# zraorg/ZRA

Hardware: AMD Instinct MI355X
Metric: compress + RA-decompress GiB/s, 16 GiB @ 64 KiB frames, 1/2/4/8 MI355X (higher is better)
Workload: dtype u8

## Files before the change

### zra_amd/csrc/zra_decode.hip

```cpp
#include "zra_dev.h"
#include "zra_kernels.h"

using namespace zra_dev;

namespace {

constexpr int DEC_THREADS = 64;
constexpr int BATCH = 64;
#ifndef ZRA_XWIN
#define ZRA_XWIN 4032
#endif
constexpr u32 XPRE = 64, XWIN = ZRA_XWIN;
constexpr u32 BLOCK_MAX = 128u << 10;

__constant__ u32 c_ll_base[36] = {0,1,2,3,4,5,6,7,8,9,10,11,12,13,14,15,16,18,20,22,24,28,32,40,48,64,128,256,512,1024,2048,4096,8192,16384,32768,65536};
__constant__ u8 c_ll_bits[36] = {0,0,0,0,0,0,0,0,0,0,0,0,0,0,0,0,1,1,1,1,2,2,3,3,4,6,7,8,9,10,11,12,13,14,15,16};
__constant__ u32 c_ml_base[53] = {3,4,5,6,7,8,9,10,11,12,13,14,15,16,17,18,19,20,21,22,23,24,25,26,27,28,29,30,31,32,33,34,
                                  35,37,39,41,43,47,51,59,67,83,99,131,259,515,1027,2051,4099,8195,16387,32771,65539};
__constant__ u8 c_ml_bits[53] = {0,0,0,0,0,0,0,0,0,0,0,0,0,0,0,0,0,0,0,0,0,0,0,0,0,0,0,0,0,0,0,0,
                                 1,1,1,1,2,2,3,3,4,4,5,7,8,9,10,11,12,13,14,15,16};
__constant__ short c_ll_defnorm[36] = {4,3,2,2,2,2,2,2,2,2,2,2,2,1,1,1,2,2,2,2,2,2,2,2,2,3,2,1,1,1,1,1,-1,-1,-1,-1};
__constant__ short c_ml_defnorm[53] = {1,4,3,2,2,2,2,2,2,1,1,1,1,1,1,1,1,1,1,1,1,1,1,1,1,1,1,1,1,1,1,1,
                                       1,1,1,1,1,1,1,1,1,1,1,1,1,1,-1,-1,-1,-1,-1,-1,-1};
__constant__ short c_of_defnorm[29] = {1,1,1,1,1,1,2,2,2,1,1,1,1,1,1,1,1,1,1,1,1,1,1,1,-1,-1,-1,-1,-1};
__constant__ u16 c_huf_t0[16][2] = {{0,0},{0,0},{38,130},{448,128},{556,128},{714,128},{883,128},{897,128},{926,128},{947,128},{1107,128},{1177,128},{1242,128},{1349,128},{1455,128},{722,128}};
__constant__ u16 c_huf_t1[16][2] = {{1,1},{1,1},{1313,74},{1353,74},{1353,74},{1418,74},{1437,74},{1515,75},{1613,75},{1729,77},{2083,81},{2379,87},{2415,93},{2644,106},{2422,124},{1891,145}};

__device__ __forceinline__ u64 mk_seqsym(u32 baseValue, u32 addBits, u32 nbBits, u32 nextBase) {
  return (u64)baseValue | ((u64)addBits << 32) | ((u64)nbBits << 40) | ((u64)nextBase << 48);
}
__device__ __forceinline__ u32 mk_cell(u32 sym, u32 addBits, u32 nbBits, u32 nextBase) {
  return sym | (addBits << 8) | (nbBits << 16) | (nextBase << 20);
}

#ifdef ZRA_SMALL_PROFILE
__device__ unsigned long long zra_small_prof[64];
extern "C" __attribute__((visibility("default"))) void ZraHipDebugReadSmallProfile(unsigned long long* out16, int reset) {
  (void)hipMemcpyFromSymbol(out16, HIP_SYMBOL(zra_small_prof), sizeof(unsigned long long) * 64);
  if (reset) { unsigned long long z[64] = {0}; (void)hipMemcpyToSymbol(HIP_SYMBOL(zra_small_prof), z, sizeof(z)); }
}
#define SPROF(k) { __builtin_amdgcn_s_waitcnt(0); const u64 n_ = __builtin_amdgcn_s_memtime(); if (lane == 0) atomicAdd(&zra_small_prof[k], n_ - spt_); spt_ = n_; }
#define SPROF_T0 u64 spt_ = __builtin_amdgcn_s_memtime();
#define SPROF_RESET spt_ = __builtin_amdgcn_s_memtime();
#else
#define SPROF(k)
#define SPROF_T0
#define SPROF_RESET
#endif
#ifdef ZRA_SMALL_PROFILE
#define PPROF_T0 u64 ppt_ = __builtin_amdgcn_s_memtime();
#define PPROF(k) if (FUSED) { __builtin_amdgcn_s_waitcnt(0); const u64 n_ = __builtin_amdgcn_s_memtime(); if (lane == 0) atomicAdd(&zra_small_prof[k], n_ - ppt_); ppt_ = n_; }
#define LPROF_T0 u64 lpt_ = __builtin_amdgcn_s_memtime();
#define LPROF(k) { __builtin_amdgcn_s_waitcnt(0); const u64 n_ = __builtin_amdgcn_s_memtime(); atomicAdd(&zra_small_prof[k], n_ - lpt_); lpt_ = n_; }
#else
#define PPROF_T0
#define PPROF(k)
#define LPROF_T0
#define LPROF(k)
#endif
constexpr u32 STAGE_BYTES = 512;
struct __attribute__((aligned(16))) ParseShared {
  u8 w0[STAGE_BYTES + 16];
  u8 w1[STAGE_BYTES + 16];
  union {
    u64 wt[64];
    u32 stage[1024];
// ... 474 lines not shown
      u32 pos = endPos;
      if (fcsHave && (fcsHi != 0 || fcsLo != produced)) err = ZE_CORRUPTION;
      if (!err && hasChecksum) { if (srcSize - pos < 4) err = ZE_CHECKSUM_WRONG; else pos += 4; }
      if (!err && pos != srcSize) err = ZE_SRCSIZE_WRONG;
    }
    if (!err) {
      const u32 p0 = a.pieceBase[j], p1 = a.pieceBase[j + 1];
      for (u32 p = p0; p < p1; p++) {
        const ZraRaPiece q = a.pieces[p];
        const u32 have = q.srcOff >= produced ? 0u : min(q.len, produced - q.srcOff);
        if (have) copy_bytes(a.raOut + q.dstOff, a.out + a.outOff[j] + q.srcOff, have, lane, nthreads);
        if (have < q.len) fill_bytes(a.raOut + q.dstOff + have, 0, q.len - have, lane, nthreads);
      }
    }
  }
}

}

namespace {
template <bool FUSED, bool ALL = false>
__device__ __forceinline__ u32 parse_job(const ZraDecodeArgs& a, const u32 j, ParseShared& S, const int lane, u32* ldsT) {
  u32 outcome = 0;
  {
    const u64 so = a.frameOff[(size_t)j * a.offStride], se = a.frameOff[(size_t)j * a.offStride + 1];
    const u8* const src = a.body + so;
    const bool spanOk = se >= so && se <= a.bodySize;
    const u32 srcSize = spanOk ? (u32)(se - so) : 0u;
    u8* const dst = a.out + a.outOff[j];
    const u32 dstCap = a.outCap[j];
    const u32 limit = a.limit ? a.limit[j] : 0xFFFFFFFFu;
    ZraDecFrame* const F = &a.frames[j];
    u32 nBlk = 0; bool bail = false;
    const u32* prevT[3] = {nullptr, nullptr, nullptr};

    auto stage = [&](u8* w, u32 pos) -> u32 {
      const u32 avail = pos < srcSize ? min(srcSize - pos, STAGE_BYTES) : 0u;
      const u32 at = 8u * (u32)lane;
      u64 v = 0;
      if (at + 8 <= avail) v = ld64(src + pos + at);
      else for (u32 k = 0; at + k < avail && k < 8; k++) v |= (u64)src[pos + at + k] << (8 * k);
      *(u64*)(w + at) = v;
      if (lane < 2) *(u64*)(w + STAGE_BYTES + 8 * lane) = 0;
      return avail;
    };
    PPROF_T0
    const u32 startPos = a.round == 0 ? 0u : F->blkPos;
    const u32 staged0 = stage(S.w0, startPos);

    if (lane == 0) {
      S.err = 0; S.frameEnd = 0; S.winPos = startPos; S.winLen = staged0;
      if (a.round == 0) {
        S.produced = 0; S.hufValid = 0; S.llValid = S.mlValid = S.ofValid = 0; S.ofShare = 0;
        S.rep[0] = 1; S.rep[1] = 4; S.rep[2] = 8;
      }
    }
    wsync();
    if (lane == 0) {
      if (a.round == 0) {
        const u8* const hsrc = S.w0;
        u32 hs = 0;
        S.fcsHave = 0; S.hasChecksum = 0; S.bigWindow = 0;
        if (!spanOk || srcSize < 9) S.err = ZE_SRCSIZE_WRONG;
        else {
          u32 fhd = hsrc[4], did = fhd & 3, ss = (fhd >> 5) & 1, fcs = fhd >> 6;
          u32 didSize = did == 3 ? 4 : did;
          u32 fcsSize = fcs == 0 ? ss : fcs == 1 ? 2 : fcs == 2 ? 4 : 8;
// ... 120 lines not shown
      {
        const u32 at = bpos + S.seqPos;
        const u32 got = stage(S.w1, at);
        (void)got;
        wsync();
      }
      const u8* const sw = S.w1 - S.seqPos;
      const u8* const swLim = S.w1 + STAGE_BYTES + 8;
      if (lane == 0) {
        parse_seq_header(S, sw + S.seqPos, bsize - S.seqPos);
        if (S.err) { S.lateErr = S.err; S.err = 0; S.nbSeq = 0; S.seqTables = 0; }
        if (S.alloc && S.nbSeq) {
          const u64 take = ((u64)S.nbSeq + 3) & ~3ull;
          const u64 at = atomicAdd((unsigned long long*)&a.counters[ZRA_DC_SEQCUR], (unsigned long long)take);
          if (at + take > a.seqCap) S.alloc = 0;
          S.seqBase = at;
        }
      }
      wsync();
      if (ALL && (!S.alloc || nBlk >= a.bpf)) { bail = true; break; }
      if (!S.alloc) {
        if (lane == 0) {
          save_persistent(S.hdrPos, produced0, hv0, hmb0, hns0, hx20);
          if (!FUSED) a.nextActive[atomicAdd(&a.counters[ZRA_DC_NNEXT], 1u)] = j;
        }
        handed = true; outcome = 2;
        wsync();
        break;
      }

      PPROF(10)
      const u32 nbSeq = S.nbSeq, regen = S.litRegen;
      const size_t jb = ALL ? (size_t)j * a.bpf + nBlk : (size_t)j;
      u32* const T = ALL ? a.blkTables + jb * ZRA_DEC_TBL_WORDS : a.tables + (size_t)j * ZRA_DEC_TBL_WORDS;
      if (S.seqTables) {
        for (int kind = 0; kind < 3; kind++) {
          const int k = kind == 0 ? 0 : kind == 1 ? 2 : 1;
          const u32 mode = k == 0 ? (S.seqModes >> 6) : k == 2 ? ((S.seqModes >> 4) & 3) : ((S.seqModes >> 2) & 3);
          if (lane == 0) {
            u32 tl = 0, ms = 0, used = 0;
            seq_table_parse(S, k, mode, sw + S.seqPos, bsize - S.seqPos, &tl, &ms, &used, swLim);
            S.seqPos += used; S.tl = tl; S.ms = ms;
            if (mode == 3) { u32 v = k == 0 ? S.llValid : k == 1 ? S.mlValid : S.ofValid; if (!v) S.err = ZE_CORRUPTION; }
            if (S.err) { S.lateErr = S.err; S.err = 0; }
          }
          wsync();
          PPROF(11)
          if (S.lateErr) break;
          const u32 tl = S.tl, ms = S.ms;
          u32* const G = T + (k == 0 ? ZRA_DEC_TBL_LL : k == 1 ? ZRA_DEC_TBL_ML : ZRA_DEC_TBL_OF);
          if (mode == 1) {
            if (lane == 0) {
              if (k == 2) { G[0] = mk_cell(ms, ms, 0, 0); S.ofShare = (ms > 22) ? 256u : 0u; }
              else G[0] = mk_cell(ms, k == 0 ? c_ll_bits[ms] : c_ml_bits[ms], 0, 0);
              if (FUSED) { u32* const GL = ldsT + (k == 0 ? ZRA_LDS_TBL_LL : k == 1 ? ZRA_LDS_TBL_ML : ZRA_LDS_TBL_OF); GL[0] = G[0]; if (k != 2) GL[1] = k == 0 ? c_ll_base[ms] : c_ml_base[ms]; }
            }
          } else if (mode != 3) {
            build_fse_dtable(S.stage, S.norm, ms, tl, k, S.spread, (u64*)S.w0, S.wnext, lane);
            wsync();
            const u32 words = (k == 2 ? 1u : 2u) << tl;
            if (!FUSED) for (u32 i = lane; i < (1u << tl); i += DEC_THREADS) G[i] = S.stage[k == 2 ? i : 2 * i];
            if (FUSED) { u32* const GL = ldsT + (k == 0 ? ZRA_LDS_TBL_LL : k == 1 ? ZRA_LDS_TBL_ML : ZRA_LDS_TBL_OF); for (u32 i = lane; i < words; i += DEC_THREADS) GL[i] = S.stage[i]; }
            if (k == 2) {
              u32 cnt = 0;
              for (u32 i = lane; i < (1u << tl); i += DEC_THREADS) cnt += (S.stage[i] & 0xFF) > 22;
              cnt = wave_sum(cnt);
              if (lane == 0) S.ofShare = cnt << (8 - tl);
            }
            wsync();
          }
          if (lane == 0 && mode != 3) {
            if (k == 0) { S.llLog = tl; S.llValid = 1; } else if (k == 1) { S.mlLog = tl; S.mlValid = 1; } else { S.ofLog = tl; S.ofValid = 1; }
          }
          if (ALL) {
            if (mode == 3 && prevT[k] && prevT[k] != G) {
              const u32 lg = k == 0 ? S.llLog : k == 1 ? S.mlLog : S.ofLog;
              for (u32 i = lane; i < (1u << lg); i += DEC_THREADS) G[i] = prevT[k][i];
            }
            prevT[k] = G;
          }
          wsync();
          PPROF(12)
        }
      }

      if (ALL) {
        ZraDecFrame* const D = &a.blkRecs[jb];
        if (lane == 0) {
          save_persistent_to(D, S.hdrPos, produced0, S.hufValid, S.hufMaxBits, S.hufNSym, S.hufX2);
          if (nBlk) { D->rep[0] = ZRA_REP_MARK(0); D->rep[1] = ZRA_REP_MARK(1); D->rep[2] = ZRA_REP_MARK(2); }
          D->bpos = bpos; D->bsize = bsize; D->blast = S.blkLast;
          D->litKind = S.litKind; D->litRegen = regen; D->litArg = S.litArg; D->litBase = S.litBase;
          D->litStreams = S.litStreams;
          for (int k = 0; k < 4; k++) { D->streamOff[k] = S.streamOff[k]; D->streamLen[k] = S.streamLen[k]; }
          D->hufErr = 0; D->lateErr = S.lateErr;
          D->nbSeq = S.lateErr ? 0u : nbSeq; D->seqPos = S.seqPos; D->seqBase = S.seqBase;
          D->longMode = 0;
          D->chainErr = 0; D->nSeqValid = 0; D->seqOut = 0; D->seqLit = 0; D->truncated = 0;
          a.pending[atomicAdd(&a.counters[ZRA_DC_NPENDING], 1u)] = (u32)jb;
          if (S.litKind == 2) a.hufJobs[atomicAdd(&a.counters[ZRA_DC_NHUF], 1u)] = (u32)jb;
          S.produced = produced0 + (S.blkLast ? 0u : ZRA_FMB_BLOCK); S.blkPos = bpos + bsize; S.frameEnd = S.blkLast;
          S.winLen = 0;
        }
        if (S.litKind == 2) {
          for (u32 i = lane; i < 256; i += DEC_THREADS) { D->weights[i] = S.weights[i]; D->hufStart[i] = S.hufStart[i]; }
        }
        if (S.lateErr) bail = true;
        nBlk++;
        wsync();
        continue;
// ... 381 lines not shown
    bc += nb; return v;
  }
  __device__ __forceinline__ u32 read_fast(u32 nb) {
    const u32 v = (u32)((c << (bc & 63)) >> ((64 - nb) & 63));
    bc += nb; return v;
  }
  __device__ __forceinline__ int reload() {
    if (bc > 64) return OVERFLOW;
    if (ptr >= 8) { ptr -= bc >> 3; bc &= 7; c = fetch(ptr); return UNFINISHED; }
    if (ptr == 0) return bc < 64 ? ENDOFBUFFER : COMPLETED;
    u32 nbBytes = bc >> 3; int r = UNFINISHED;
    if (ptr < nbBytes) { nbBytes = ptr; r = ENDOFBUFFER; }
    ptr -= nbBytes; bc -= nbBytes * 8; c = fetch(ptr);
    return r;
  }
  __device__ __forceinline__ void reload_quiet(bool wide, const u8* pad) {
    const u32 nb = bc <= 64 ? min(bc >> 3, ptr) : 0u;
    ptr -= nb; bc -= nb * 8;
    const u64 v = RING ? fetch(ptr) : ld64(wide ? base + ptr : pad);
    c = nb ? v : c;
  }
};
typedef ZdsT<false> Zds;

}

namespace {
template <bool LDSTAB>
__device__ __forceinline__ void chain_body(const ZraDecodeArgs& a, u32* const ldsTabs, u32* const baseLL, u32* const baseML, u32* const ldsRings = nullptr) {
  const int lane = threadIdx.x;
  const u32 nPend = a.counters[ZRA_DC_NPENDING];
  bool have = false, drained = false;
  ZraDecFrame* F = nullptr;
  const u32* T = nullptr;
  u64* sq = nullptr;
  ZdsT<LDSTAB> br; br.c = 0; br.bc = 0; br.ptr = 0; br.base = nullptr; br.ring = nullptr; br.rLo = 0;
  br.lim = a.body + a.bodySize; br.pf = make_uint4(0, 0, 0, 0); br.pfState = 0; br.pfAge = 0;
  if (LDSTAB) br.ring = (u8*)(ldsRings + (u32)lane * CHAIN_RING_WORDS);
  u32 sLL = 0, sOF = 0, sML = 0, rep0 = 1, rep1 = 4, rep2 = 8;
  u32 i = 0, nbSeq = 0, outPos = 0, litPos = 0, outCap = 0, regen = 0, produced0 = 0, limit = 0;
  u32 longMode = 0, err = 0, jErr = 0xFFFFFFFFu, valid = 0, validOut = 0, validLit = 0, truncated = 0;
  u64 q0 = 0, q1 = 0, q2 = 0;
  u32 eL = 0, eM = 0, eO = 0;
  bool wide = false; const u8* pad = nullptr;
  bool fresh = false; u32 freshJob = 0;
  const u16* const cells16 = (const u16*)ldsTabs + (size_t)lane * ZRA_DEC_TBL_WORDS;
  u32 logLL = 0, logML = 0, logOF = 0;
  auto fetch_cells = [&]() {
    if (LDSTAB) { eL = cells16[ZRA_DEC_TBL_LL + sLL]; eM = cells16[ZRA_DEC_TBL_ML + sML]; eO = cells16[ZRA_DEC_TBL_OF + sOF]; }
    else { eL = T[ZRA_DEC_TBL_LL + sLL]; eM = T[ZRA_DEC_TBL_ML + sML]; eO = T[ZRA_DEC_TBL_OF + sOF]; }
  };
  auto c_code = [&](u32 e) -> u32 { return e & 63u; };
  auto c_sbits = [&](u32 e, u32 lg) -> u32 { if (LDSTAB) return lg - (31u - (u32)__builtin_clz(e >> 6)); return (e >> 16) & 0xF; };
  auto c_sbase = [&](u32 e, u32 lg) -> u32 {
    if (LDSTAB) { const u32 v = e >> 6, hb = 31u - (u32)__builtin_clz(v); return (v ^ (1u << hb)) << (lg - hb); }
    return e >> 20;
  };
  baseLL[lane] = lane < 36 ? c_ll_base[lane] | (LDSTAB ? (u32)c_ll_bits[lane] << 24 : 0u) : 0u;
  baseML[lane] = lane < 53 ? c_ml_base[lane] | (LDSTAB ? (u32)c_ml_bits[lane] << 24 : 0u) : 0u;
  wsync();
  if (LDSTAB && (u32)lane >= ZRA_CHAIN_LDS_FRAMES) drained = true;

  auto finish = [&]() {
    { const u32 r = valid & 3u, b = valid - r;
      if (r >= 1) sq[b] = q0;
      if (r >= 2) sq[b + 1] = q1;
      if (r >= 3) sq[b + 2] = q2; }
    if (!err && !truncated) {
      if (regen - litPos > outCap - outPos) err = ZE_DSTSIZE_TOOSMALL;
    }
    F->chainErr = err; F->nSeqValid = valid; F->seqOut = validOut; F->seqLit = validLit; F->truncated = truncated;
    F->repOut[0] = rep0; F->repOut[1] = rep1; F->repOut[2] = rep2;
    have = false;
  };

  for (;;) {
    const u64 want = __ballot(!have && !drained);
    if (want) {
      u32 base = 0;
      const u32 cnt = (u32)__builtin_popcountll(want);
      if (lane == (int)__builtin_ctzll(want)) base = atomicAdd(&a.counters[ZRA_DC_QCHAIN], cnt);
      base = bcast_u32(base, (u32)__builtin_ctzll(want));
      if (!have && !drained) {
        const u32 idx = base + (u32)__builtin_popcountll(want & ((1ull << lane) - 1ull));
        if (idx >= nPend) drained = true;
        else {
          const u32 j = a.pending[idx];
          const size_t gj = frame_of(a, j);
          F = &a.frames[j];
          T = a.tables + (size_t)j * ZRA_DEC_TBL_WORDS;
          const u8* const blk = a.body + a.frameOff[gj * a.offStride] + F->bpos;
          nbSeq = F->nbSeq; regen = F->litRegen; produced0 = F->produced; longMode = F->longMode;
          outCap = a.outCap[gj] - produced0;
          limit = a.limit ? a.limit[gj] : 0xFFFFFFFFu;
          sq = a.seqs + F->seqBase;
          rep0 = F->rep[0]; rep1 = F->rep[1]; rep2 = F->rep[2];
          i = 0; outPos = 0; litPos = 0; err = 0; jErr = 0xFFFFFFFFu; valid = 0; validOut = 0; validLit = 0; truncated = 0;
          have = true; br.rLo = 0; br.pfState = 0;
          if (F->hufErr) { err = ZE_CORRUPTION; nbSeq = 0; finish(); }
          else if (F->lateErr) { err = F->lateErr; nbSeq = 0; finish(); }
          else if (nbSeq) {
            if (!br.init(blk + F->seqPos, F->bsize - F->seqPos)) { err = ZE_CORRUPTION; finish(); }
            else {
              logLL = F->llLog; logOF = F->ofLog; logML = F->mlLog;
              sLL = br.read(logLL); br.reload();
              sOF = br.read(logOF); br.reload();
              sML = br.read(logML); br.reload();
              wide = F->bsize - F->seqPos >= 8;
              pad = a.body + a.frameOff[gj * a.offStride];
              if (LDSTAB) { fresh = true; freshJob = j; } else fetch_cells();
            }
          }
        }
      }
    }
    if (LDSTAB) {
      u64 nm = __ballot(fresh);
      while (nm) {
        const u32 l = (u32)__builtin_ctzll(nm); nm &= nm - 1;
        const u32 jj = bcast_u32(freshJob, l);
        const uint4* const g4 = (const uint4*)(a.tables + (size_t)jj * ZRA_DEC_TBL_WORDS);
        uint2* const d2 = (uint2*)((u16*)ldsTabs + (size_t)l * ZRA_DEC_TBL_WORDS);
        const ZraDecFrame* const Fj = &a.frames[jj];
        const u32 lgL = Fj->llLog, lgM = Fj->mlLog, lgO = Fj->ofLog;
        for (u32 i = (u32)lane; i < ZRA_DEC_TBL_WORDS / 4; i += DEC_THREADS) {
          const uint4 q = g4[i];
          const u32 lg = 4 * i < ZRA_DEC_TBL_ML ? lgL : 4 * i < ZRA_DEC_TBL_OF ? lgM : lgO;
          auto pk = [&](u32 x) -> u32 { const u32 nb = min((x >> 16) & 0xFu, lg); return (x & 63u) | (((1u << (lg - nb)) | ((x >> 20) >> nb)) << 6); };
          d2[i] = make_uint2(pk(q.x) | (pk(q.y) << 16), pk(q.z) | (pk(q.w) << 16));
        }
      }
      if (__ballot(fresh)) wsync();
      if (fresh) { fetch_cells(); fresh = false; }
    }
    if (!__ballot(have)) break;

    if (have) {
      bool go = true;
      if (LDSTAB) { br.ring_guard(); br.ring_advance(); }
      if (i >= nbSeq) {
        if (!err && nbSeq && !longMode && br.reload() < Zds::COMPLETED) err = ZE_CORRUPTION;
        finish(); go = false;
      } else if (longMode) {
        if (br.reload() > Zds::COMPLETED) {
          if (jErr == 0xFFFFFFFFu || i <= jErr + 4) err = ZE_CORRUPTION;
          finish(); go = false;
        } else if (jErr != 0xFFFFFFFFu && i > jErr + 4) { finish(); go = false; }
      }
      if (go) {
        u32 ll = baseLL[c_code(eL)], ml = baseML[c_code(eM)], off;
        const u32 ofBits = LDSTAB ? c_code(eO) : (eO >> 8) & 0xFF, mlBits = LDSTAB ? ml >> 24 : (eM >> 8) & 0xFF, llBits = LDSTAB ? ll >> 24 : (eL >> 8) & 0xFF;
        if (LDSTAB) { ll &= 0xFFFFFFu; ml &= 0xFFFFFFu; }
        bool badOff = false;
        if (ofBits > 1) {
          off = ((1u << ofBits) - 3u) + br.read_fast(ofBits);
          if (a.bpf > 1 && off >= ZRA_REP_MARK_LO) badOff = true;
          rep2 = rep1; rep1 = rep0; rep0 = off;
        } else {
          const u32 ll0 = (ll == 0);
          if (ofBits == 0) {
            if (!ll0) off = rep0;
            else { off = rep1; rep1 = rep0; rep0 = off; }
          } else {
            const u32 idx = 1 + ll0 + br.read_fast(1);
            u32 t = idx == 3 ? rep0 - 1 : idx == 1 ? rep1 : rep2;
            t += !t;
            if (idx != 1) rep2 = rep1;
            rep1 = rep0; rep0 = off = t;
          }
        }
        if (mlBits) ml += br.read_fast(mlBits);
        if (llBits + mlBits + ofBits >= 57 - (9 + 9 + 8)) br.reload();
        if (llBits) ll += br.read_fast(llBits);
        sLL = c_sbase(eL, logLL) + br.read(c_sbits(eL, logLL));
        sML = c_sbase(eM, logML) + br.read(c_sbits(eM, logML));
        sOF = c_sbase(eO, logOF) + br.read(c_sbits(eO, logOF));
        fetch_cells();
        if (!longMode) br.reload_quiet(wide, pad);
        if (jErr == 0xFFFFFFFFu) {
          u32 e = 0;
          if (ll + ml > outCap - outPos) e = ZE_DSTSIZE_TOOSMALL;
          else if (ll > regen - litPos) e = ZE_CORRUPTION;
          else if (badOff || (off > produced0 + outPos + ll && !(a.bpf > 1 && off >= ZRA_REP_MARK_LO))) e = ZE_CORRUPTION;
          if (e) { jErr = i; err = e; if (!longMode) finish(); }
          else {
            const u64 qv = (u64)ll | ((u64)ml << 18) | ((u64)min(off, 0x0FFFFFFFu) << 36);
            const u32 slot = i & 3u;
            if (slot == 0) q0 = qv; else if (slot == 1) q1 = qv; else if (slot == 2) q2 = qv;
            else { uint4* d4 = (uint4*)(sq + (i - 3)); d4[0] = make_uint4((u32)q0, (u32)(q0 >> 32), (u32)q1, (u32)(q1 >> 32)); d4[1] = make_uint4((u32)q2, (u32)(q2 >> 32), (u32)qv, (u32)(qv >> 32)); }
            outPos += ll + ml; litPos += ll;
            valid = i + 1; validOut = outPos; validLit = litPos;
            if (produced0 + outPos >= limit) { truncated = 1; finish(); }
          }
        }
        i++;
      }
    }
  }
}
}

extern "C" __global__ void __launch_bounds__(DEC_THREADS)
zra_dec_chain_kernel(ZraDecodeArgs a) {
  __shared__ u32 baseLL[64], baseML[64];
  chain_body<false>(a, nullptr, baseLL, baseML);
}
extern "C" __global__ void __launch_bounds__(DEC_THREADS)
zra_dec_chain_lds_kernel(ZraDecodeArgs a) {
  extern __shared__ u32 chainLds[];
  chain_body<true>(a, chainLds + 128, chainLds, chainLds + 64, chainLds + 128 + ZRA_CHAIN_LDS_FRAMES * (ZRA_DEC_TBL_WORDS / 2));
}

namespace {
struct __attribute__((aligned(16))) ExecShared {
  union {
    u8 slot[BATCH][64];
    u8 win[XPRE + XWIN];
  };
  u32 endAt[BATCH];
  u32 matchAt[BATCH];
  u32 job;
};
}

#ifdef ZRA_DEC_PROFILE
__device__ unsigned long long zra_dec_prof[16];
#define XCNT(k, v) { if (lane == 0) atomicAdd(&zra_dec_prof[k], (unsigned long long)(v)); }
#define XTIME(k) { __builtin_amdgcn_s_waitcnt(0); const u64 n_ = __builtin_amdgcn_s_memtime(); if (lane == 0) atomicAdd(&zra_dec_prof[k], n_ - xpt_); xpt_ = n_; }
extern "C" __attribute__((visibility("default"))) void ZraHipDebugReadDecProfile(unsigned long long* out16, int reset) {
  (void)hipMemcpyFromSymbol(out16, HIP_SYMBOL(zra_dec_prof), sizeof(unsigned long long) * 16);
  if (reset) { unsigned long long z[16] = {0}; (void)hipMemcpyToSymbol(HIP_SYMBOL(zra_dec_prof), z, sizeof(z)); }
}
#else
#define XCNT(k, v)
#define XTIME(k)
#endif

namespace {
struct ExecCtx {
  u8* out; const u8* lit; u32 litKind; u8 rleByte;
  u32 outBase, litBase;
  const u8* src; u32 srcSize, produced0, regen;
  bool preValid;
// ... 632 lines not shown
```

### zra_amd/csrc/zra_engine.hip

```cpp
#include "zra_engine.h"
#include "zra_dev.h"
#include "zra_format.h"
#include "zra_env.h"
#include <algorithm>
#include <atomic>
#include <cstdio>
#include <chrono>
#include <cstdio>
#include <cstdlib>
#include <cstring>

extern "C" __global__ void zra_dec_parse_kernel(ZraDecodeArgs a);
extern "C" __global__ void zra_dec_huf_kernel(ZraDecodeArgs a);
extern "C" __global__ void zra_dec_chain_kernel(ZraDecodeArgs a);
extern "C" __global__ void zra_dec_chain_lds_kernel(ZraDecodeArgs a);
extern "C" __global__ void zra_dec_exec_kernel(ZraDecodeArgs a);
extern "C" __global__ void zra_dec_parse_all_kernel(ZraDecodeArgs a);
extern "C" __global__ void zra_dec_exec_all_kernel(ZraDecodeArgs a);
extern "C" __global__ void zra_ra_small_kernel(ZraDecodeArgs a, uint32_t* bail, const uint32_t* expect, uint32_t jobBase, unsigned long long* result);

using namespace zra_dev;

namespace zra_fmt {
uint32_t crc32(uint32_t crc, const void* data, size_t n) {
// ... 310 lines not shown
  HIPCHK(hipMemcpyAsync(two, result_.p, 16, hipMemcpyDeviceToHost, stream_));
  mark("queued rest");
  HIPCHK(hipStreamSynchronize(stream_));
  mark("sync");
  HIPCHK(hipGetLastError());
  if (hipMemsetAsync(a.counters, 0, ZRA_DC_WORDS * 4, stream_) == hipSuccess) decCountersClean_ = true;
  two[1] = 0xFFFFFFFFull - (two[1] & 0xFFFFFFFFull);
  *bailed = (uint32_t)two[1];
  if (!*bailed) *hResult = two[0];
  float ms = 0;
  if (hipEventElapsedTime(&ms, ev0_, ev1_) == hipSuccess) { lastKernelMs_ = ms; kstats_[4] += ms; kstats_[5] += 1; dstats_[5] += ms; dstats_[6] += 1; }
  return ok();
}

hipEvent_t Engine::stage_event() {
  if (stageEvNext_ == stageEv_.size()) { hipEvent_t e = nullptr; if (hipEventCreate(&e) != hipSuccess) return nullptr; stageEv_.push_back(e); }
  return stageEv_[stageEvNext_++];
}

Status Engine::decode_launch(const ZraDecodeArgs& a0, const uint32_t* dExpect, uint32_t maxFrameBytes, uint32_t jobBase, unsigned long long* hResult) {
  ZraDecodeArgs a = a0;
  const uint32_t n = a.nFrames;
  { Status st = decode_scratch(a, maxFrameBytes); if (st.zra) return st; }
  decCountersClean_ = false;
  uint32_t* listA = decLists_.as<uint32_t>(); uint32_t* listB = listA + n;
  if (!decOccParse_) {
    HIPCHK(hipOccupancyMaxActiveBlocksPerMultiprocessor(&decOccParse_, zra_dec_parse_kernel, 64, 0));
    HIPCHK(hipOccupancyMaxActiveBlocksPerMultiprocessor(&decOccExec_, zra_dec_exec_kernel, 64, 0));
    HIPCHK(hipOccupancyMaxActiveBlocksPerMultiprocessor(&decOccHuf_, zra_dec_huf_kernel, 64, 0));
    decOccParse_ = std::max(1, decOccParse_); decOccExec_ = std::max(1, decOccExec_); decOccHuf_ = std::max(1, decOccHuf_);
  }
  const int perCUParse = decOccParse_, perCUExec = decOccExec_;
  HIPCHK(hipEventRecord(ev0_, stream_));
  constexpr uint32_t chainWaves = 2;
  static const uint32_t chainLdsMin = (uint32_t)zra_env::env_int("ZRA_DEC_CHAIN_LDS_MIN", numCUs_ * 96);
  static const int chainLdsMode = zra_env::env_int("ZRA_DEC_CHAIN_LDS", 1);
  static const bool chainLdsOn = chainLdsMode != 0;
  constexpr uint32_t aheadCap = 16;
  if (!roundN_.reserve(4 * (aheadCap + 2) + 64)) return zerr(64);
  auto run_rounds = [&](ZraDecodeArgs& x, uint32_t nActive, const uint32_t* active, uint32_t round, uint32_t* lA, uint32_t* lB, uint32_t ahead) -> Status {
    uint32_t* const dN = roundN_.as<uint32_t>();
    while (nActive) {
      const uint32_t burst = std::max(1u, std::min(ahead, aheadCap));
      std::vector<hipEvent_t> evs;
      for (uint32_t bi = 0; bi < burst; bi++) {
        HIPCHK(hipMemsetAsync(x.counters, 0, ZRA_DC_WORDS * 4, stream_));
        x.active = active; x.nActive = nActive; x.round = round + bi;
        x.nActivePtr = bi ? dN + bi : nullptr;
        x.nextActive = (active == lA) ? lB : lA;
        const uint32_t gridParse = (uint32_t)std::min<uint64_t>(nActive, (uint64_t)numCUs_ * perCUParse);
        const uint32_t gridChain = (uint32_t)std::min<uint64_t>((nActive + 63) / 64, (uint64_t)numCUs_ * chainWaves);
        const uint32_t gridExec = (uint32_t)std::min<uint64_t>(nActive, (uint64_t)numCUs_ * perCUExec);
        hipEvent_t se[5];
        for (auto& e : se) { e = stage_event(); if (!e) return zerr(1); evs.push_back(e); }
        HIPCHK(hipEventRecord(se[0], stream_));
        hipLaunchKernelGGL(zra_dec_parse_kernel, dim3(gridParse), dim3(64), 0, stream_, x);
        HIPCHK(hipEventRecord(se[1], stream_));
        hipLaunchKernelGGL(zra_dec_huf_kernel, dim3((uint32_t)std::min<uint64_t>((nActive + ZRA_HUF_FRAMES - 1) / ZRA_HUF_FRAMES, (uint64_t)numCUs_ * decOccHuf_)), dim3(64), 0, stream_, x);
        HIPCHK(hipEventRecord(se[2], stream_));
        bool forked = false;
        if (chainLdsOn && nActive >= chainLdsMin) {
          if (!pipeStreams_[1]) { if (hipStreamCreateWithFlags(&pipeStreams_[1], hipStreamNonBlocking) != hipSuccess) { pipeStreams_[1] = nullptr; (void)hipGetLastError(); } }
          const size_t ldsBytes = (128 + (size_t)ZRA_CHAIN_LDS_FRAMES * (ZRA_DEC_TBL_WORDS / 2 + ZRA_CHAIN_RING_WORDS)) * 4;
          if (pipeStreams_[1] && !chainLdsAttr_) {
            if (hipFuncSetAttribute((const void*)zra_dec_chain_lds_kernel, hipFuncAttributeMaxDynamicSharedMemorySize, (int)ldsBytes) == hipSuccess) chainLdsAttr_ = 1;
            else { chainLdsAttr_ = -1; (void)hipGetLastError(); }
          }
          if (pipeStreams_[1] && chainLdsAttr_ > 0) {
            hipEvent_t eJoin = stage_event(); if (!eJoin) return zerr(1);
            HIPCHK(hipStreamWaitEvent(pipeStreams_[1], se[2], 0));
            hipLaunchKernelGGL(zra_dec_chain_lds_kernel, dim3((uint32_t)numCUs_), dim3(64), ldsBytes, pipeStreams_[1], x);
            HIPCHK(hipEventRecord(eJoin, pipeStreams_[1]));
            if (chainLdsMode != 2) hipLaunchKernelGGL(zra_dec_chain_kernel, dim3(gridChain), dim3(64), 0, stream_, x);
            HIPCHK(hipStreamWaitEvent(stream_, eJoin, 0));
            forked = true;
          }
        }
        if (!forked) hipLaunchKernelGGL(zra_dec_chain_kernel, dim3(gridChain), dim3(64), 0, stream_, x);
        HIPCHK(hipEventRecord(se[3], stream_));
        hipLaunchKernelGGL(zra_dec_exec_kernel, dim3(gridExec), dim3(64), 0, stream_, x);
        HIPCHK(hipEventRecord(se[4], stream_));
        HIPCHK(hipMemcpyAsync(dN + bi + 1, x.counters + ZRA_DC_NNEXT, 4, hipMemcpyDeviceToDevice, stream_));
        active = x.nextActive;
      }
      uint32_t next = 0;
      HIPCHK(hipMemcpyAsync(&next, dN + burst, 4, hipMemcpyDeviceToHost, stream_));
      HIPCHK(hipStreamSynchronize(stream_));
      HIPCHK(hipGetLastError());
      for (uint32_t bi = 0; bi < burst; bi++)
        for (int k = 0; k < 4; k++) { float m = 0; if (hipEventElapsedTime(&m, evs[5 * bi + k], evs[5 * bi + k + 1]) == hipSuccess) dstats_[k] += m; }
      dstats_[4] += burst;
      stageEvNext_ = 0;
      x.nActivePtr = nullptr;
      nActive = next; round += burst; ahead = 1;
      if (round > (1u << 20)) return zerr(1);
    }
// ... 4 lines not shown
  const uint32_t bpf = (uint32_t)(((uint64_t)maxFrameBytes + ZRA_FMB_BLOCK - 1) / ZRA_FMB_BLOCK);
  bool fmb = fmbEnv != 0 && bpf >= 2 && maxFrameBytes <= (64u << 20) && n >= fmbMin && (uint64_t)n * bpf < (1ull << 30);
  uint32_t nRest = n;
  if (fmb) {
    const uint64_t nb = (uint64_t)n * bpf;
    const uint64_t litAll = std::max<uint64_t>((uint64_t)n * ((uint64_t)maxFrameBytes + 16) / 2, 1u << 20);
    const uint64_t seqAll = std::max<uint64_t>((uint64_t)n * ((uint64_t)maxFrameBytes + 16) * 3 / 32, 1u << 20);
    if (!decBlkRecs_.reserve((size_t)nb * sizeof(ZraDecFrame)) || !decBlkTables_.reserve((size_t)nb * ZRA_DEC_TBL_WORDS * 4) ||
        !decBlkLists_.reserve((size_t)(2 * nb + n) * 4 + 64) || !decLits_.reserve(litAll + 64) || !decSeqs_.reserve(seqAll * 8 + 64)) {
      (void)hipGetLastError();
      fmb = false;
    }
    a.lits = decLits_.as<uint8_t>(); a.seqs = decSeqs_.as<uint64_t>();
    if (fmb) {
      ZraDecodeArgs x = a;
      x.bpf = bpf; x.blkRecs = decBlkRecs_.as<ZraDecFrame>(); x.blkTables = decBlkTables_.as<uint32_t>();
      uint32_t* bl = decBlkLists_.as<uint32_t>();
      x.pending = bl; x.hufJobs = bl + nb; x.execList = bl + 2 * nb;
      x.litCap = litAll; x.seqCap = seqAll;
      x.active = nullptr; x.nActive = n; x.round = 0; x.nActivePtr = nullptr; x.nextActive = listA;
      HIPCHK(hipMemsetAsync(x.counters, 0, ZRA_DC_WORDS * 4, stream_));
      hipEvent_t se[5];
      for (auto& e : se) { e = stage_event(); if (!e) return zerr(1); }
      HIPCHK(hipEventRecord(se[0], stream_));
      hipLaunchKernelGGL(zra_dec_parse_all_kernel, dim3((uint32_t)std::min<uint64_t>(n, (uint64_t)numCUs_ * perCUParse)), dim3(64), 0, stream_, x);
      HIPCHK(hipEventRecord(se[1], stream_));
      ZraDecodeArgs y = x; y.frames = x.blkRecs; y.tables = x.blkTables;
      hipLaunchKernelGGL(zra_dec_huf_kernel, dim3((uint32_t)std::min<uint64_t>((nb + ZRA_HUF_FRAMES - 1) / ZRA_HUF_FRAMES, (uint64_t)numCUs_ * decOccHuf_)), dim3(64), 0, stream_, y);
      HIPCHK(hipEventRecord(se[2], stream_));
      const uint32_t gridChain = (uint32_t)std::min<uint64_t>((nb + 63) / 64, (uint64_t)numCUs_ * chainWaves);
      bool forked = false;
      if (chainLdsOn && nb >= chainLdsMin) {
        if (!pipeStreams_[1]) { if (hipStreamCreateWithFlags(&pipeStreams_[1], hipStreamNonBlocking) != hipSuccess) { pipeStreams_[1] = nullptr; (void)hipGetLastError(); } }
        const size_t ldsBytes = (128 + (size_t)ZRA_CHAIN_LDS_FRAMES * (ZRA_DEC_TBL_WORDS / 2 + ZRA_CHAIN_RING_WORDS)) * 4;
        if (pipeStreams_[1] && !chainLdsAttr_) {
          if (hipFuncSetAttribute((const void*)zra_dec_chain_lds_kernel, hipFuncAttributeMaxDynamicSharedMemorySize, (int)ldsBytes) == hipSuccess) chainLdsAttr_ = 1;
          else { chainLdsAttr_ = -1; (void)hipGetLastError(); }
        }
        if (pipeStreams_[1] && chainLdsAttr_ > 0) {
          hipEvent_t eJoin = stage_event(); if (!eJoin) return zerr(1);
          HIPCHK(hipStreamWaitEvent(pipeStreams_[1], se[2], 0));
          hipLaunchKernelGGL(zra_dec_chain_lds_kernel, dim3((uint32_t)numCUs_), dim3(64), ldsBytes, pipeStreams_[1], y);
          HIPCHK(hipEventRecord(eJoin, pipeStreams_[1]));
          if (chainLdsMode != 2) hipLaunchKernelGGL(zra_dec_chain_kernel, dim3(gridChain), dim3(64), 0, stream_, y);
          HIPCHK(hipStreamWaitEvent(stream_, eJoin, 0));
          forked = true;
        }
      }
      if (!forked) hipLaunchKernelGGL(zra_dec_chain_kernel, dim3(gridChain), dim3(64), 0, stream_, y);
      HIPCHK(hipEventRecord(se[3], stream_));
      hipLaunchKernelGGL(zra_dec_exec_all_kernel, dim3((uint32_t)std::min<uint64_t>(n, (uint64_t)numCUs_ * perCUExec)), dim3(64), 0, stream_, x);
      HIPCHK(hipEventRecord(se[4], stream_));
      uint32_t back = 0;
      HIPCHK(hipMemcpyAsync(&back, x.counters + ZRA_DC_NNEXT, 4, hipMemcpyDeviceToHost, stream_));
      HIPCHK(hipStreamSynchronize(stream_));
      HIPCHK(hipGetLastError());
      for (int k = 0; k < 4; k++) { float m = 0; if (hipEventElapsedTime(&m, se[k], se[k + 1]) == hipSuccess) dstats_[k] += m; }
      dstats_[4] += 1;
      stageEvNext_ = 0;
      nRest = back;
    }
  }
  Status st = fmb ? run_rounds(a, nRest, listA, 0, listA, listB, 1)
                  : run_rounds(a, n, nullptr, 0, listA, listB, (maxFrameBytes + (128u << 10) - 1) / (128u << 10));
  if (st.zra) return st;
  HIPCHK(hipEventRecord(ev1_, stream_));
  const uint32_t tb = 256;
// ... 296 lines not shown
```

### zra_amd/csrc/zra_kernels.h

```cpp
#pragma once
#include <stdint.h>
#include <stddef.h>

#ifndef ZRA_HUF_FRAMES
#define ZRA_HUF_FRAMES 2
#endif
#define ZRA_DEC_TBL_LL 0u
#define ZRA_DEC_TBL_ML 512u
#define ZRA_DEC_TBL_OF 1024u
#define ZRA_DEC_TBL_WORDS 1280u
#define ZRA_LDS_TBL_LL 0u
#define ZRA_LDS_TBL_ML 1024u
#define ZRA_LDS_TBL_OF 2048u
#define ZRA_LDS_TBL_WORDS 2304u
#define ZRA_CHAIN_LDS_FRAMES 59u
#define ZRA_CHAIN_RING_WORDS 36u

struct ZraDecFrame {
  uint32_t blkPos, produced, done;
  uint32_t hufValid, hufMaxBits, hufNSym, hufX2;
  uint32_t llValid, mlValid, ofValid, llLog, mlLog, ofLog, ofShare;
  uint32_t rep[3];
  uint32_t fcsLo, fcsHi, fcsHave, hasChecksum, bigWindow;
  uint32_t bpos, bsize, blast;
  uint32_t litKind, litRegen, litArg;
  uint32_t litStreams, streamOff[4], streamLen[4];
  uint32_t hufErr, lateErr;
  uint32_t nbSeq, seqPos, longMode;
  uint64_t litBase, seqBase;
  uint32_t chainErr, nSeqValid, seqOut, seqLit, truncated;
  uint32_t repOut[3];
  uint32_t nBlk, endPos, parseTrunc, pad1_;
  alignas(8) uint8_t weights[256];
  alignas(8) uint16_t hufStart[256];
};
#define ZRA_REP_MARK_LO 0x0C000000u
#define ZRA_REP_MARK(k) (ZRA_REP_MARK_LO + ((uint32_t)(k) << 24) + 0x00800000u)
#define ZRA_FMB_BLOCK (128u << 10)

struct ZraRaPiece { uint64_t dstOff; uint32_t srcOff, len; };

struct ZraDecodeArgs {
  const uint8_t* body;
  uint64_t bodySize;
  const uint64_t* frameOff;
  uint32_t offStride;
  uint8_t* out;
// ... 161 lines not shown
```

Baseline: 20.68.

## Store decode FSE tables as packed two-byte cells in global memory

The parse stage now writes the global per-frame FSE decode tables as 16-bit packed cells (code plus a leading-one encoding of width and base), halving ZRA_DEC_TBL_WORDS. The chain kernel's LDS fill becomes a straight 128-bit copy with no repacking, and the non-LDS path decodes cells the same way as the LDS path. The aim is to cut table write/read bandwidth and the per-frame repack cost. The trade-off is extra clz/shift work on the global-table path. A header with static_asserts checks that the encoding round-trips.

```diff
diff --git a/zra_amd/csrc/zra_decode.hip b/zra_amd/csrc/zra_decode.hip
--- a/zra_amd/csrc/zra_decode.hip
+++ b/zra_amd/csrc/zra_decode.hip
@@ -1,5 +1,6 @@
 #include "zra_dev.h"
 #include "zra_kernels.h"
+#include "zra_fse_cell.h"
 
 using namespace zra_dev;
 
@@ -32,6 +33,7 @@
 __device__ __forceinline__ u32 mk_cell(u32 sym, u32 addBits, u32 nbBits, u32 nextBase) {
   return sym | (addBits << 8) | (nbBits << 16) | (nextBase << 20);
 }
+__device__ __forceinline__ u32 cell16_of(u32 c, u32 tableLog) { return zra_cell::pack(c & 63u, (c >> 16) & 0xFu, c >> 20, tableLog); }
 
 #ifdef ZRA_SMALL_PROFILE
 __device__ unsigned long long zra_small_prof[64];
@@ -572,7 +574,7 @@
     const u32 limit = a.limit ? a.limit[j] : 0xFFFFFFFFu;
     ZraDecFrame* const F = &a.frames[j];
     u32 nBlk = 0; bool bail = false;
-    const u32* prevT[3] = {nullptr, nullptr, nullptr};
+    const u16* prevT[3] = {nullptr, nullptr, nullptr};
 
     auto stage = [&](u8* w, u32 pos) -> u32 {
       const u32 avail = pos < srcSize ? min(srcSize - pos, STAGE_BYTES) : 0u;
@@ -759,7 +761,7 @@
       PPROF(10)
       const u32 nbSeq = S.nbSeq, regen = S.litRegen;
       const size_t jb = ALL ? (size_t)j * a.bpf + nBlk : (size_t)j;
-      u32* const T = ALL ? a.blkTables + jb * ZRA_DEC_TBL_WORDS : a.tables + (size_t)j * ZRA_DEC_TBL_WORDS;
+      u16* const T = (u16*)(ALL ? a.blkTables + jb * ZRA_DEC_TBL_WORDS : a.tables + (size_t)j * ZRA_DEC_TBL_WORDS);
       if (S.seqTables) {
         for (int kind = 0; kind < 3; kind++) {
           const int k = kind == 0 ? 0 : kind == 1 ? 2 : 1;
@@ -775,18 +777,22 @@
           PPROF(11)
           if (S.lateErr) break;
           const u32 tl = S.tl, ms = S.ms;
-          u32* const G = T + (k == 0 ? ZRA_DEC_TBL_LL : k == 1 ? ZRA_DEC_TBL_ML : ZRA_DEC_TBL_OF);
+          u16* const G = T + (k == 0 ? ZRA_DEC_TBL_LL : k == 1 ? ZRA_DEC_TBL_ML : ZRA_DEC_TBL_OF);
           if (mode == 1) {
             if (lane == 0) {
-              if (k == 2) { G[0] = mk_cell(ms, ms, 0, 0); S.ofShare = (ms > 22) ? 256u : 0u; }
-              else G[0] = mk_cell(ms, k == 0 ? c_ll_bits[ms] : c_ml_bits[ms], 0, 0);
-              if (FUSED) { u32* const GL = ldsT + (k == 0 ? ZRA_LDS_TBL_LL : k == 1 ? ZRA_LDS_TBL_ML : ZRA_LDS_TBL_OF); GL[0] = G[0]; if (k != 2) GL[1] = k == 0 ? c_ll_base[ms] : c_ml_base[ms]; }
+              const u32 c1 = mk_cell(ms, k == 2 ? ms : k == 0 ? c_ll_bits[ms] : c_ml_bits[ms], 0, 0);
+              if (k == 2) S.ofShare = (ms > 22) ? 256u : 0u;
+              if (!FUSED) G[0] = (u16)cell16_of(c1, 0);
+              if (FUSED) { u32* const GL = ldsT + (k == 0 ? ZRA_LDS_TBL_LL : k == 1 ? ZRA_LDS_TBL_ML : ZRA_LDS_TBL_OF); GL[0] = c1; if (k != 2) GL[1] = k == 0 ? c_ll_base[ms] : c_ml_base[ms]; }
             }
           } else if (mode != 3) {
             build_fse_dtable(S.stage, S.norm, ms, tl, k, S.spread, (u64*)S.w0, S.wnext, lane);
             wsync();
             const u32 words = (k == 2 ? 1u : 2u) << tl;
-            if (!FUSED) for (u32 i = lane; i < (1u << tl); i += DEC_THREADS) G[i] = S.stage[k == 2 ? i : 2 * i];
+            if (!FUSED) {
+              const u32 st = k == 2 ? 1u : 2u;
+              for (u32 i = lane; i < (1u << tl) / 2; i += DEC_THREADS) ((u32*)G)[i] = cell16_of(S.stage[2 * i * st], tl) | (cell16_of(S.stage[(2 * i + 1) * st], tl) << 16);
+            }
             if (FUSED) { u32* const GL = ldsT + (k == 0 ? ZRA_LDS_TBL_LL : k == 1 ? ZRA_LDS_TBL_ML : ZRA_LDS_TBL_OF); for (u32 i = lane; i < words; i += DEC_THREADS) GL[i] = S.stage[i]; }
             if (k == 2) {
               u32 cnt = 0;
@@ -802,7 +808,7 @@
           if (ALL) {
             if (mode == 3 && prevT[k] && prevT[k] != G) {
               const u32 lg = k == 0 ? S.llLog : k == 1 ? S.mlLog : S.ofLog;
-              for (u32 i = lane; i < (1u << lg); i += DEC_THREADS) G[i] = prevT[k][i];
+              for (u32 i = lane; i < max((1u << lg) / 2, 1u); i += DEC_THREADS) ((u32*)G)[i] = ((const u32*)prevT[k])[i];
             }
             prevT[k] = G;
           }
@@ -1250,7 +1256,7 @@
   const u32 nPend = a.counters[ZRA_DC_NPENDING];
   bool have = false, drained = false;
   ZraDecFrame* F = nullptr;
-  const u32* T = nullptr;
+  const u16* T = nullptr;
   u64* sq = nullptr;
   ZdsT<LDSTAB> br; br.c = 0; br.bc = 0; br.ptr = 0; br.base = nullptr; br.ring = nullptr; br.rLo = 0;
   br.lim = a.body + a.bodySize; br.pf = make_uint4(0, 0, 0, 0); br.pfState = 0; br.pfAge = 0;
@@ -1262,20 +1268,17 @@
   u32 eL = 0, eM = 0, eO = 0;
   bool wide = false; const u8* pad = nullptr;
   bool fresh = false; u32 freshJob = 0;
-  const u16* const cells16 = (const u16*)ldsTabs + (size_t)lane * ZRA_DEC_TBL_WORDS;
-  u32 logLL = 0, logML = 0, logOF = 0;
+  const u16* const cells16 = (const u16*)ldsTabs + (size_t)lane * ZRA_DEC_TBL_CELLS;
+  u32 logLL = 0, logML = 0, logOF = 0, logs = 0;
+  auto lg_ll = [&]() -> u32 { return LDSTAB ? logLL : logs & 15u; };
+  auto lg_ml = [&]() -> u32 { return LDSTAB ? logML : (logs >> 4) & 15u; };
+  auto lg_of = [&]() -> u32 { return LDSTAB ? logOF : logs >> 8; };
   auto fetch_cells = [&]() {
-    if (LDSTAB) { eL = cells16[ZRA_DEC_TBL_LL + sLL]; eM = cells16[ZRA_DEC_TBL_ML + sML]; eO = cells16[ZRA_DEC_TBL_OF + sOF]; }
-    else { eL = T[ZRA_DEC_TBL_LL + sLL]; eM = T[ZRA_DEC_TBL_ML + sML]; eO = T[ZRA_DEC_TBL_OF + sOF]; }
+    const u16* const c = LDSTAB ? cells16 : T;
+    eL = c[ZRA_DEC_TBL_LL + sLL]; eM = c[ZRA_DEC_TBL_ML + sML]; eO = c[ZRA_DEC_TBL_OF + sOF];
   };
-  auto c_code = [&](u32 e) -> u32 { return e & 63u; };
-  auto c_sbits = [&](u32 e, u32 lg) -> u32 { if (LDSTAB) return lg - (31u - (u32)__builtin_clz(e >> 6)); return (e >> 16) & 0xF; };
-  auto c_sbase = [&](u32 e, u32 lg) -> u32 {
-    if (LDSTAB) { const u32 v = e >> 6, hb = 31u - (u32)__builtin_clz(v); return (v ^ (1u << hb)) << (lg - hb); }
-    return e >> 20;
-  };
-  baseLL[lane] = lane < 36 ? c_ll_base[lane] | (LDSTAB ? (u32)c_ll_bits[lane] << 24 : 0u) : 0u;
-  baseML[lane] = lane < 53 ? c_ml_base[lane] | (LDSTAB ? (u32)c_ml_bits[lane] << 24 : 0u) : 0u;
+  baseLL[lane] = lane < 36 ? c_ll_base[lane] | ((u32)c_ll_bits[lane] << 24) : 0u;
+  baseML[lane] = lane < 53 ? c_ml_base[lane] | ((u32)c_ml_bits[lane] << 24) : 0u;
   wsync();
   if (LDSTAB && (u32)lane >= ZRA_CHAIN_LDS_FRAMES) drained = true;
 
@@ -1306,7 +1309,7 @@
           const u32 j = a.pending[idx];
           const size_t gj = frame_of(a, j);
           F = &a.frames[j];
-          T = a.tables + (size_t)j * ZRA_DEC_TBL_WORDS;
+          T = (const u16*)(a.tables + (size_t)j * ZRA_DEC_TBL_WORDS);
           const u8* const blk = a.body + a.frameOff[gj * a.offStride] + F->bpos;
           nbSeq = F->nbSeq; regen = F->litRegen; produced0 = F->produced; longMode = F->longMode;
           outCap = a.outCap[gj] - produced0;
@@ -1324,6 +1327,7 @@
               sLL = br.read(logLL); br.reload();
               sOF = br.read(logOF); br.reload();
               sML = br.read(logML); br.reload();
+              if (!LDSTAB) logs = logLL | (logML << 4) | (logOF << 8);
               wide = F->bsize - F->seqPos >= 8;
               pad = a.body + a.frameOff[gj * a.offStride];
               if (LDSTAB) { fresh = true; freshJob = j; } else fetch_cells();
@@ -1338,15 +1342,8 @@
         const u32 l = (u32)__builtin_ctzll(nm); nm &= nm - 1;
         const u32 jj = bcast_u32(freshJob, l);
         const uint4* const g4 = (const uint4*)(a.tables + (size_t)jj * ZRA_DEC_TBL_WORDS);
-        uint2* const d2 = (uint2*)((u16*)ldsTabs + (size_t)l * ZRA_DEC_TBL_WORDS);
-        const ZraDecFrame* const Fj = &a.frames[jj];
-        const u32 lgL = Fj->llLog, lgM = Fj->mlLog, lgO = Fj->ofLog;
-        for (u32 i = (u32)lane; i < ZRA_DEC_TBL_WORDS / 4; i += DEC_THREADS) {
-          const uint4 q = g4[i];
-          const u32 lg = 4 * i < ZRA_DEC_TBL_ML ? lgL : 4 * i < ZRA_DEC_TBL_OF ? lgM : lgO;
-          auto pk = [&](u32 x) -> u32 { const u32 nb = min((x >> 16) & 0xFu, lg); return (x & 63u) | (((1u << (lg - nb)) | ((x >> 20) >> nb)) << 6); };
-          d2[i] = make_uint2(pk(q.x) | (pk(q.y) << 16), pk(q.z) | (pk(q.w) << 16));
-        }
+        u32* const d = ldsTabs + (size_t)l * ZRA_DEC_TBL_WORDS;
+        for (u32 i = (u32)lane; i < ZRA_DEC_TBL_WORDS / 4; i += DEC_THREADS) lds_st128((u8*)(d + 4 * i), g4[i]);
       }
       if (__ballot(fresh)) wsync();
       if (fresh) { fetch_cells(); fresh = false; }
@@ -1366,9 +1363,9 @@
         } else if (jErr != 0xFFFFFFFFu && i > jErr + 4) { finish(); go = false; }
       }
       if (go) {
-        u32 ll = baseLL[c_code(eL)], ml = baseML[c_code(eM)], off;
-        const u32 ofBits = LDSTAB ? c_code(eO) : (eO >> 8) & 0xFF, mlBits = LDSTAB ? ml >> 24 : (eM >> 8) & 0xFF, llBits = LDSTAB ? ll >> 24 : (eL >> 8) & 0xFF;
-        if (LDSTAB) { ll &= 0xFFFFFFu; ml &= 0xFFFFFFu; }
+        u32 ll = baseLL[zra_cell::code(eL)], ml = baseML[zra_cell::code(eM)], off;
+        const u32 ofBits = zra_cell::code(eO), mlBits = ml >> 24, llBits = ll >> 24;
+        ll &= 0xFFFFFFu; ml &= 0xFFFFFFu;
         bool badOff = false;
         if (ofBits > 1) {
           off = ((1u << ofBits) - 3u) + br.read_fast(ofBits);
@@ -1390,9 +1387,9 @@
         if (mlBits) ml += br.read_fast(mlBits);
         if (llBits + mlBits + ofBits >= 57 - (9 + 9 + 8)) br.reload();
         if (llBits) ll += br.read_fast(llBits);
-        sLL = c_sbase(eL, logLL) + br.read(c_sbits(eL, logLL));
-        sML = c_sbase(eM, logML) + br.read(c_sbits(eM, logML));
-        sOF = c_sbase(eO, logOF) + br.read(c_sbits(eO, logOF));
+        sLL = zra_cell::base(eL, lg_ll()) + br.read(zra_cell::width(eL, lg_ll()));
+        sML = zra_cell::base(eM, lg_ml()) + br.read(zra_cell::width(eM, lg_ml()));
+        sOF = zra_cell::base(eO, lg_of()) + br.read(zra_cell::width(eO, lg_of()));
         fetch_cells();
         if (!longMode) br.reload_quiet(wide, pad);
         if (jErr == 0xFFFFFFFFu) {
@@ -1426,7 +1423,7 @@
 extern "C" __global__ void __launch_bounds__(DEC_THREADS)
 zra_dec_chain_lds_kernel(ZraDecodeArgs a) {
   extern __shared__ u32 chainLds[];
-  chain_body<true>(a, chainLds + 128, chainLds, chainLds + 64, chainLds + 128 + ZRA_CHAIN_LDS_FRAMES * (ZRA_DEC_TBL_WORDS / 2));
+  chain_body<true>(a, chainLds + 128, chainLds, chainLds + 64, chainLds + 128 + ZRA_CHAIN_LDS_FRAMES * ZRA_DEC_TBL_WORDS);
 }
 
 namespace {
diff --git a/zra_amd/csrc/zra_engine.hip b/zra_amd/csrc/zra_engine.hip
--- a/zra_amd/csrc/zra_engine.hip
+++ b/zra_amd/csrc/zra_engine.hip
@@ -366,7 +366,7 @@
   }
   const int perCUParse = decOccParse_, perCUExec = decOccExec_;
   HIPCHK(hipEventRecord(ev0_, stream_));
-  constexpr uint32_t chainWaves = 2;
+  constexpr uint32_t chainWaves = ZRA_CHAIN_WAVES;
   static const uint32_t chainLdsMin = (uint32_t)zra_env::env_int("ZRA_DEC_CHAIN_LDS_MIN", numCUs_ * 96);
   static const int chainLdsMode = zra_env::env_int("ZRA_DEC_CHAIN_LDS", 1);
   static const bool chainLdsOn = chainLdsMode != 0;
@@ -395,7 +395,7 @@
         bool forked = false;
         if (chainLdsOn && nActive >= chainLdsMin) {
           if (!pipeStreams_[1]) { if (hipStreamCreateWithFlags(&pipeStreams_[1], hipStreamNonBlocking) != hipSuccess) { pipeStreams_[1] = nullptr; (void)hipGetLastError(); } }
-          const size_t ldsBytes = (128 + (size_t)ZRA_CHAIN_LDS_FRAMES * (ZRA_DEC_TBL_WORDS / 2 + ZRA_CHAIN_RING_WORDS)) * 4;
+          const size_t ldsBytes = (128 + (size_t)ZRA_CHAIN_LDS_FRAMES * (ZRA_DEC_TBL_WORDS + ZRA_CHAIN_RING_WORDS)) * 4;
           if (pipeStreams_[1] && !chainLdsAttr_) {
             if (hipFuncSetAttribute((const void*)zra_dec_chain_lds_kernel, hipFuncAttributeMaxDynamicSharedMemorySize, (int)ldsBytes) == hipSuccess) chainLdsAttr_ = 1;
             else { chainLdsAttr_ = -1; (void)hipGetLastError(); }
@@ -466,7 +466,7 @@
       bool forked = false;
       if (chainLdsOn && nb >= chainLdsMin) {
         if (!pipeStreams_[1]) { if (hipStreamCreateWithFlags(&pipeStreams_[1], hipStreamNonBlocking) != hipSuccess) { pipeStreams_[1] = nullptr; (void)hipGetLastError(); } }
-        const size_t ldsBytes = (128 + (size_t)ZRA_CHAIN_LDS_FRAMES * (ZRA_DEC_TBL_WORDS / 2 + ZRA_CHAIN_RING_WORDS)) * 4;
+        const size_t ldsBytes = (128 + (size_t)ZRA_CHAIN_LDS_FRAMES * (ZRA_DEC_TBL_WORDS + ZRA_CHAIN_RING_WORDS)) * 4;
         if (pipeStreams_[1] && !chainLdsAttr_) {
           if (hipFuncSetAttribute((const void*)zra_dec_chain_lds_kernel, hipFuncAttributeMaxDynamicSharedMemorySize, (int)ldsBytes) == hipSuccess) chainLdsAttr_ = 1;
           else { chainLdsAttr_ = -1; (void)hipGetLastError(); }
diff --git a/zra_amd/csrc/zra_fse_cell.h b/zra_amd/csrc/zra_fse_cell.h
--- /dev/null
+++ b/zra_amd/csrc/zra_fse_cell.h
@@ -0,0 +1,45 @@
+#pragma once
+#include <stdint.h>
+
+#if defined(__HIPCC__) || defined(__CUDACC__)
+#define ZRA_CELL_FN __host__ __device__ constexpr
+#else
+#define ZRA_CELL_FN constexpr
+#endif
+
+namespace zra_cell {
+
+constexpr uint32_t CODE_BITS = 6, CODE_MASK = 63;
+
+ZRA_CELL_FN uint32_t pack(uint32_t code, uint32_t width, uint32_t base, uint32_t tableLog) {
+  return code | (((1u << (tableLog - width)) | (base >> width)) << CODE_BITS);
+}
+ZRA_CELL_FN uint32_t code(uint32_t cell) { return cell & CODE_MASK; }
+ZRA_CELL_FN uint32_t top(uint32_t cell) { return 31u - (uint32_t)__builtin_clz(cell >> CODE_BITS); }
+ZRA_CELL_FN uint32_t width(uint32_t cell, uint32_t tableLog) { return tableLog - top(cell); }
+ZRA_CELL_FN uint32_t base(uint32_t cell, uint32_t tableLog) {
+  const uint32_t v = cell >> CODE_BITS, hb = top(cell);
+  return (v ^ (1u << hb)) << (tableLog - hb);
+}
+
+ZRA_CELL_FN bool round_trips(uint32_t c, uint32_t w, uint32_t b, uint32_t lg) {
+  const uint32_t e = pack(c, w, b, lg);
+  return e < 65536u && code(e) == c && width(e, lg) == w && base(e, lg) == b;
+}
+ZRA_CELL_FN bool proves_table_log(uint32_t lg) {
+  for (uint32_t w = 0; w <= lg; w++)
+    for (uint32_t b = 0; b < (1u << lg); b += 1u << w)
+      if (!round_trips(0, w, b, lg) || !round_trips(CODE_MASK, w, b, lg)) return false;
+  return true;
+}
+ZRA_CELL_FN bool proves_codes() {
+  for (uint32_t c = 0; c <= CODE_MASK; c++)
+    if (!round_trips(c, 3, 8 * 37, 9) || !round_trips(c, 0, 0, 0)) return false;
+  return true;
+}
+static_assert(proves_table_log(0), "two-byte FSE cell: one-symbol table");
+static_assert(proves_table_log(5) && proves_table_log(6) && proves_table_log(7) && proves_table_log(8) && proves_table_log(9),
+              "two-byte FSE cell: unpack(pack(x)) != x");
+static_assert(proves_codes(), "two-byte FSE cell: code field");
+
+}
diff --git a/zra_amd/csrc/zra_kernels.h b/zra_amd/csrc/zra_kernels.h
--- a/zra_amd/csrc/zra_kernels.h
+++ b/zra_amd/csrc/zra_kernels.h
@@ -8,11 +8,15 @@
 #define ZRA_DEC_TBL_LL 0u
 #define ZRA_DEC_TBL_ML 512u
 #define ZRA_DEC_TBL_OF 1024u
-#define ZRA_DEC_TBL_WORDS 1280u
+#define ZRA_DEC_TBL_CELLS 1280u
+#define ZRA_DEC_TBL_WORDS 640u
 #define ZRA_LDS_TBL_LL 0u
 #define ZRA_LDS_TBL_ML 1024u
 #define ZRA_LDS_TBL_OF 2048u
 #define ZRA_LDS_TBL_WORDS 2304u
+#ifndef ZRA_CHAIN_WAVES
+#define ZRA_CHAIN_WAVES 2u
+#endif
 #define ZRA_CHAIN_LDS_FRAMES 59u
 #define ZRA_CHAIN_RING_WORDS 36u
 
```

Result: no change. 20.65 (-0.2%).
